# ziatdinovmax/pyroVED

Measured on AMD Instinct MI355X. Metric: images/sec (SVI step), higher is better.
Workload: dtype bf16; 1 GPU; C2 iVAE 28x28 invariances=['r','t'] latent_dim=2 bernoulli, batch 256 per GPU (global 256), bf16 MFMA operands for the hidden-layer contractions (fp32 accumulate; fp32 elsewhere); the guide (fc encoder, sample, split) runs in the decoder launch's prologue in fp32, SVI step = ELBO+grads+Adam; parallelism=dp1

## Files before the change

### pyroved_amd/csrc/pv_elementwise.hip

```cpp
#include "pv_common.h"
#include "pv_kernels.h"
#include "pv_wgrad_small.h"
#include "pv_side.h"
#include "pv_sdec_fused.h"

#define LOG_SQRT_2PI 0.91893853320467274178f
#define BERN_EPS 1.1920928955078125e-07f

__device__ __forceinline__ float block_sum_256(float v, float* sm ) {
  v = pv_wave_sum(v);
  pv_lds_barrier();
  if ((threadIdx.x & 63) == 0) sm[threadIdx.x >> 6] = v;
  pv_lds_barrier();
  return (sm[0] + sm[1]) + (sm[2] + sm[3]);
}

__global__ __launch_bounds__(256) void pv_head_fwd_kernel(PvHead h) {
  __shared__ float sm[4];
  const int total = h.B * h.z_dim;
  float lp = 0.0f, lq = 0.0f;
  for (int e = threadIdx.x; e < total; e += 256) {
    const int b = e / h.z_dim, i = e % h.z_dim;
    const int ldh = h.ldh > 0 ? h.ldh : 2 * h.z_dim;
    const float mu = h.head[(int64_t)b * ldh + i];
// ... 994 lines not shown
}

int pv_latent_bwd_reduce(const PvLatentBwd& p, const float* part, int grid, float* G, const PvFusedOffsets& o, int cd,
                         hipStream_t s, int fmt) {
  if (p.H > 512 || p.lat_in > 64 + (p.K > 0 ? p.K : 0) || p.hb.z_dim > 256 || p.K > 128) return PV_EINVAL;
  PV_LAUNCH_FORK(pv_latent_bwd_reduce_kernel, dim3(pv_fused_reduce_blocks(fmt) + p.hb.B), dim3(256), 0, s, p, part, grid, G, o, cd, fmt);
  PV_LAUNCH_CHECK();
  return 0;
}

__global__ __launch_bounds__(256) void pv_rec_wgrad_kernel(const float* __restrict__ part, int G_, float* __restrict__ Gr, PvFusedOffsets o,
                                                           int cd, int fmt, PvWgradSmall w, PvRecAdam ra, int rwx) {
  __shared__ f32x4 smr[4][64];
  __shared__ float wpart[WG_WAVES][16][17];
  __shared__ float wrpart[WG_WAVES][16];
  const int nred = pv_fused_reduce_blocks(fmt), id = (int)blockIdx.x;
  if (id < nred) { if (!(rwx & 1)) pv_sdec_fused_reduce_block(part, G_, Gr, o, cd, 0, id, smr, fmt, (rwx & 4) ? PvRecAdam{} : ra); return; }
  if (rwx & 2) return;
  pv_wgrad_small_block(w, id - nred, (int)gridDim.x - nred, wpart, wrpart);
}

int pv_rec_wgrad(const float* part, int grid, float* G, const PvFusedOffsets& o, int cd, int fmt, const PvGemm* gs, int n,
                 const PvAdamFuse* adam, const PvFinishArgs* fin, hipStream_t s, unsigned* tick) {
  PvWgradSmall w;
  int guests = 0;
  const int tiles = pv_wgrad_small_fill(w, gs, n, adam, fin, &guests);
  if (tiles < 0) return tiles;
  const int fin_blocks = (fin && fin->scalars) ? 1 : 0;
  if (tick && !fin_blocks) return PV_EINVAL;
  w.tick = tick;
  PvRecAdam ra{};
// ... 114 lines not shown
```

### pyroved_amd/csrc/pv_plan.hip

```cpp
#include "pv_common.h"
#include <algorithm>
#include <stdlib.h>
#include "pv_kernels.h"
#include "pv_sdec_fused.h"
#include "pv_linear.h"
#include "pv_convstack.h"
#include "pv_side.h"
#include "pv_conv.h"

namespace {

struct Carver {
  char* base;
  int64_t off;
  float* take(int64_t nfloats) {
    float* p = base ? (float*)(base + off) : nullptr;
    off += pv_align_up(nfloats * (int64_t)sizeof(float), 256);
    return p;
  }
};

}

int64_t gemm_ws_need(int64_t M, int64_t N, int64_t K) {
// ... 805 lines not shown
  hb.head = L.enc_ext ? p->ext_head : L.head; hb.dhead = L.enc_ext ? p->ext_dhead : L.dhead;
  hb.scale_direct = L.enc_ext ? 1 : 0;
  hb.B = (int)B; hb.z_dim = (int)z; hb.coord_dim = p->coord_dim;
  hb.has_r = p->has_r; hb.has_t = p->has_t; hb.has_s = p->has_s;
  hb.tp0 = p->t_prior[0]; hb.tp1 = p->t_prior[1]; hb.sc_prior = p->sc_prior; hb.beta = p->beta;
  hb.ldh = L.enc_ext ? 0 : (int)plan_head_w(p); hb.kl_mode = p->kl_mode;
  lb.K = (int)K; lb.alpha = L.alpha; lb.beta_disc = p->beta_disc;
  hb.w = p->row_w; lb.row_ll = p->row_elbo ? L.row_ll : nullptr; lb.dzc_out = p->dy ? L.dzc : nullptr;
  static const int chain_env = pv_exp_int("PV_CHAIN", 1) ? 1 : 0;
  const bool chain = chain_env && L.enc_compact && !L.enc_ext && 2 * z + K <= 256;
  if (chain) {
    lb.enc_n = p->n_enc; lb.enc_params = p->params; lb.enc_head = p->head;
    for (int i = 0; i < p->n_enc; ++i) { lb.enc_l[i] = p->enc[i]; lb.enc_act[i] = L.eact[i]; lb.enc_dp[i] = L.edp[i]; }
  }
  static const int ab_tail = pv_exp_int("PV_FOLD_CHAIN", 1);
  const int rec_fmt = p->fused >= 2 ? pv_sdec_fused_bf16_record_fmt(p->fused == 2, R / FD_UNIT, p->dec_kernel) : PV_REC_ROWMAJOR;
  const PvGemm wz = wgrad_problem(L.dhz, H, zin, ldz, G + p->fc_latent.w_off, G + p->fc_coord.b_off, S, lat_in, H);
  PvGemm tail_probs[4];
  int tail_np = -1;
  if (ab_tail && want_grads && chain && f.part_rs && f.dhz_out && f.dzc_out && K == 0 && H == FD_H && !p->row_w &&
      p->kl_mode == PV_KL_SAMPLED &&
      !p->row_elbo && !p->dy && p->head.out_dim <= 16 && p->n_enc == 2 && p->enc[0].out_dim == FD_H && p->enc[1].in_dim == FD_H &&
      p->enc[1].out_dim == FD_H && p->head.in_dim == FD_H) {
    tail_np = compact_wgrad_problems(p, L, &wz, 1, tail_probs);
    if (tail_np > 0 && adam) {
      auto lsz = [](const pv_layer& l) { return (int64_t)l.in_dim * l.out_dim + (l.b_off >= 0 ? l.out_dim : 0); };
      int64_t want = lsz(p->head) + lsz(p->fc_coord) + lsz(p->fc_latent) + lsz(p->out);
      for (int i = 0; i < p->n_enc; ++i) want += lsz(p->enc[i]);
      for (int i = 0; i < p->n_dec; ++i) want += lsz(p->dec[i]);
      int64_t cov = 2 * (int64_t)H * H + (int64_t)H * (3 + p->coord_dim) + 1;
      for (int i = 0; i < tail_np; ++i) cov += (int64_t)tail_probs[i].M * tail_probs[i].N + (tail_probs[i].rowsumA ? tail_probs[i].M : 0);
// ... 465 lines not shown
```

### pyroved_amd/csrc/pv_sdec_fused.h

```cpp
#pragma once
#include "pv_common.h"

#define FD_H 128
#define FD_UNIT 16
#define FD_WAVES 8
#define FD_REC (2 * FD_H * FD_H + 14 * FD_H)
#define PV_RS_W 8
#define FB_WIMG_BYTES (4 * FD_H * FD_H * 2 + 256)

struct PvFused {
  const float* x;
  const float* grid;
  const float* tp;
  const float* hz;
  float hz_scale;
  const float *Wc, *bc;
  const float *W1, *b1;
  const float *W2, *b2;
  const float *wo, *bo;
  float* llrow;
  float* loc;
  float* rowtp;
  float* part_hz;
  float* part_rs;
// ... 70 lines not shown
int pv_sdec_fused_w8x3_launch(const PvFused& f, int grid, bool grads, hipStream_t s, int waves);
int64_t pv_sdec_fused_w8x3_park_bytes(int grid);
int pv_sdec_fused_w8h_launch(const PvFused& f, int grid, bool ds, hipStream_t s);
int64_t pv_sdec_fused_bf16_park_bytes(bool x3, int64_t units, int grid, int sel);
int pv_sdec_fused_bf16_waves(bool x3, int64_t units, int sel);
int pv_sdec_fused_bf16_record_fmt(bool x3, int64_t units, int sel);
bool pv_sdec_fused_sel_valid(int fused, int sel);
struct PvFusedOffsets { int64_t W1, b1, W2, b2, Wc, wo, bo; };
int pv_sdec_fused_reduce(const float* part, int grid, float* G, const PvFusedOffsets& o, int cd, int dwo_slots,
                         hipStream_t s);

#define PV_FUSED_REDUCE_BLOCKS (((2 * FD_H * FD_H + 5 * FD_H + 1 + 3) / 4 + 63) / 64)
#define PV_REC_ROWMAJOR 0
#define PV_REC_LANE_F32 1
#define PV_REC_LANE_BF16 2
#define PV_FUSED_REDUCE_VEC_BLOCKS (((5 * FD_H + 1 + 3) / 4 + 63) / 64)
#define PV_FUSED_REDUCE_MAT_BLOCKS_F32 ((2 * FD_H * FD_H / 4) / 64)
#define PV_FUSED_REDUCE_MAT_BLOCKS_BF16 ((2 * (FD_H / 2) * FD_H / 4) / 64)
__host__ __device__ inline int pv_fused_reduce_mat_blocks(int fmt) {
  return fmt == PV_REC_LANE_BF16 ? PV_FUSED_REDUCE_MAT_BLOCKS_BF16 : PV_FUSED_REDUCE_MAT_BLOCKS_F32;
}
__host__ __device__ inline int pv_fused_reduce_blocks(int fmt) {
  return fmt == PV_REC_ROWMAJOR ? PV_FUSED_REDUCE_BLOCKS : pv_fused_reduce_mat_blocks(fmt) + PV_FUSED_REDUCE_VEC_BLOCKS;
}
#ifndef PV_RED_UNROLL
#define PV_RED_UNROLL 8
#endif
struct PvRecAdam { PvAdamFuse a; int on; };
__device__ __forceinline__ void pv_rec_out(float* __restrict__ Gr, int idx, float v, const PvRecAdam& ad) {
  if (ad.on) pv_adam_update(ad.a.p, ad.a.g, ad.a.m, ad.a.v, (Gr - ad.a.g) + idx, v, ad.a.b1, ad.a.b2, ad.a.eps, ad.a.step_size, ad.a.bc2_sqrt);
  else Gr[idx] = v;
}
template <int FMT>
__device__ __forceinline__ void pv_sdec_fused_reduce_block_lane(const float* __restrict__ part, int G_, float* __restrict__ Gr,
                                                                const PvFusedOffsets& o, int block, f32x4 (*sm)[64],
                                                                const PvRecAdam& ad = PvRecAdam{}) {
  const int c = threadIdx.x & 63, sl = threadIdx.x >> 6;
  const int per = (G_ + 3) / 4;
  const int w0 = sl * per, w1 = min(G_, w0 + per);
  const float* pbase = part + 4 * (block * 64 + c);
  f32x4 a = {0.0f, 0.0f, 0.0f, 0.0f}, b = {0.0f, 0.0f, 0.0f, 0.0f};
  if (FMT == PV_REC_LANE_BF16) {
    typedef unsigned int u32x4_ __attribute__((ext_vector_type(4)));
#pragma unroll PV_RED_UNROLL
    for (int w = w0; w < w1; ++w) {
      const u32x4_ v = *reinterpret_cast<const u32x4_*>(pbase + (int64_t)w * FD_REC);
      a[0] += __uint_as_float(v[0] << 16); a[1] += __uint_as_float(v[0] & 0xffff0000u);
      a[2] += __uint_as_float(v[1] << 16); a[3] += __uint_as_float(v[1] & 0xffff0000u);
      b[0] += __uint_as_float(v[2] << 16); b[1] += __uint_as_float(v[2] & 0xffff0000u);
      b[2] += __uint_as_float(v[3] << 16); b[3] += __uint_as_float(v[3] & 0xffff0000u);
    }
  } else {
#pragma unroll PV_RED_UNROLL
    for (int w = w0; w < w1; ++w) a += *reinterpret_cast<const f32x4*>(pbase + (int64_t)w * FD_REC);
  }
  sm[sl][c] = a;
  __syncthreads();
  const f32x4 ta = (sm[0][c] + sm[1][c]) + (sm[2][c] + sm[3][c]);
  f32x4 tb = b;
  if (FMT == PV_REC_LANE_BF16) {
    __syncthreads();
    sm[sl][c] = b;
    __syncthreads();
    tb = (sm[0][c] + sm[1][c]) + (sm[2][c] + sm[3][c]);
  }
  if (sl != 0) return;
  const int r = c & 15, q = c >> 4;
  if (FMT == PV_REC_LANE_BF16) {
    const int oo = block & 3, s_ = (block >> 2) & 1, wave = block >> 3, jp = wave >> 1, kh = wave & 1;
    const int row0 = 32 * jp + 16 * (s_ ^ kh) + 4 * q, col = 64 * kh + 16 * oo + r;
#pragma unroll
    for (int i = 0; i < 4; ++i) {
      pv_rec_out(Gr, o.W1 + (row0 + i) * FD_H + col, ta[i], ad);
      pv_rec_out(Gr, o.W2 + (row0 + i) * FD_H + col, tb[i], ad);
    }
  } else {
    const int kb = block & 7, s_ = (block >> 3) & 1, wave = (block >> 4) & 3, m = block >> 6;
    const int row0 = 16 * (2 * wave + s_) + 4 * q, col = 16 * kb + r;
    const int dst = m == 0 ? o.W1 : o.W2;
#pragma unroll
    for (int i = 0; i < 4; ++i) pv_rec_out(Gr, dst + (row0 + i) * FD_H + col, ta[i], ad);
  }
}
__device__ __forceinline__ void pv_sdec_fused_reduce_block(const float* __restrict__ part, int G_,
                                                           float* __restrict__ Gr, const PvFusedOffsets& o, int cd,
                                                           int dwo_slots, int block, f32x4 (*sm)[64], int fmt = PV_REC_ROWMAJOR,
                                                           const PvRecAdam& ad = PvRecAdam{}) {
  const int HH = FD_H * FD_H;
  const int total = 2 * HH + 5 * FD_H + 1;
  const int c = threadIdx.x & 63, sl = threadIdx.x >> 6;
  if (fmt != PV_REC_ROWMAJOR && block < pv_fused_reduce_mat_blocks(fmt)) {
    if (fmt == PV_REC_LANE_BF16) pv_sdec_fused_reduce_block_lane<PV_REC_LANE_BF16>(part, G_, Gr, o, block, sm, ad);
    else pv_sdec_fused_reduce_block_lane<PV_REC_LANE_F32>(part, G_, Gr, o, block, sm, ad);
    return;
  }
  const int e = fmt != PV_REC_ROWMAJOR ? 2 * HH + ((block - pv_fused_reduce_mat_blocks(fmt)) * 64 + c) * 4 : (block * 64 + c) * 4;
  const int per = (G_ + 3) / 4;
  const int w0 = sl * per, w1 = min(G_, w0 + per);
  f32x4 v = {0.0f, 0.0f, 0.0f, 0.0f};
  if (e < total) {
    const bool slots = dwo_slots && e >= 2 * HH + 4 * FD_H && e < 2 * HH + 5 * FD_H;
    if (slots) {
      for (int w = w0; w < w1; ++w) {
        const float* p8 = part + (int64_t)w * FD_REC + 2 * HH + 6 * FD_H + (e - (2 * HH + 4 * FD_H));
        f32x4 a = {0.0f, 0.0f, 0.0f, 0.0f};
        for (int k = 0; k < FD_WAVES; ++k) a += *reinterpret_cast<const f32x4*>(p8 + k * FD_H);
        v += a;
// ... 31 lines not shown
```

### pyroved_amd/csrc/pv_sdec_fused_w8.hip

```cpp
#include "pv_sdec_fused.h"
#include "pv_fb_layout.h"
#include "pv_kernels.h"
#include <stdlib.h>

typedef short short4_ __attribute__((ext_vector_type(4)));
typedef short short8_ __attribute__((ext_vector_type(8)));
typedef __attribute__((address_space(3))) short4_ lds_short4;

#define W8_WAVES 8
#define W8_ROWS (W8_WAVES * FD_UNIT)
#define W8_THREADS (64 * W8_WAVES)
#define LDS2 144
#define W8_ARR (W8_ROWS * LDS2)
#define W8_ARR_BYTES (2 * W8_ARR)
#define WO_W1 0
#define WO_W2 IMG_BYTES
#define WO_SA (2 * IMG_BYTES)
#define WO_SB (WO_SA + W8_ARR_BYTES)
#define WO_VEC (WO_SB + W8_ARR_BYTES)
#define WO_ATAB (WO_VEC + 3 * FD_H * 4)
#define WO_TTAB (WO_ATAB + 8 * 64 * 8)
#define WO_INFO (WO_TTAB + 4 * 64 * 16)
#define WO_RED (WO_INFO + 3 * W8_ROWS * 4)
#define WO_CHZ (WO_RED + 256)
// ... 349 lines not shown
  return h;
}
__device__ __forceinline__ f32x4 w8_mul_dtanh4(const f32x4& d, const bf16x4& hb) {
  const f32x4 t = w8_f32_of(hb);
  return d * (t * t - 1.0f);
}

#define WF_H1 WO_SA
#define WF_H2 (WF_H1 + 512)
#define WF_HD (WF_H2 + 512)
#define WF_P (WF_HD + 512)
#define WF_P_WAVE (64 * 17 * 4)
static_assert(WF_P + W8_WAVES * WF_P_WAVE <= WO_VEC, "guide scratch fits in the staging arrays");
#include "pv_gemv16.h"

#define W8_COOP_SPINS 4096
__device__ unsigned w8_coop_late_total;
extern "C" int pv_debug_coop_late_count(unsigned* out) {
  return (int)hipMemcpyFromSymbol(out, HIP_SYMBOL(w8_coop_late_total), sizeof(unsigned));
}
template <bool GRADS, int LIK, int FOLDK>
__global__ __launch_bounds__(W8_THREADS) void pv_sdec_w8_kernel(PvFused f, PvEncFold e) {
  constexpr bool FOLD = FOLDK != 0, CHAIN = FOLDK >= 2, COOP = FOLDK == 3;
  extern __shared__ __attribute__((aligned(16))) char smb[];
  const int tid = threadIdx.x, lane0 = tid & 63, lane = lane0, r = lane & 15, q = lane >> 4;
  const int wave = __builtin_amdgcn_readfirstlane(tid >> 6);
  const int g = blockIdx.x, G = gridDim.x;
  const unsigned lds0 = __builtin_amdgcn_readfirstlane((unsigned)(size_t)smb);
  const __bf16* W1h = reinterpret_cast<const __bf16*>(smb + WO_W1);
  const __bf16* W2h = reinterpret_cast<const __bf16*>(smb + WO_W2);
// ... 359 lines not shown
  const int xun = (int)f.x_units;
  struct Pos { int unit, b, loc, xu; };
  auto pos_of = [&](int unit_) {
    Pos p_;
    p_.unit = unit_; p_.b = unit_ / upb; p_.loc = unit_ - p_.b * upb; p_.xu = xun > 0 ? unit_ % xun : unit_;
    return p_;
  };
  auto advance = [&](Pos& p_, int by) {
    p_.unit += by; p_.loc += by; p_.xu += by;
    while (p_.loc >= upb) { p_.loc -= upb; ++p_.b; }
    if (xun > 0) { while (p_.xu >= xun) p_.xu -= xun; }
  };
  const bool has_tail = W8_TAIL && ((u_hi - u_lo) & (W8_WAVES - 1)) == 1;
  const int u_end = has_tail ? u_hi - 1 : u_hi;
  const Pos pos_lo = pos_of(has_tail ? u_end : u_lo);
  Pos pos_cur = pos_of(u_lo + wave < u_end ? u_lo + wave : (has_tail ? u_end : u_lo));
  Pos pos_nx = pos_cur;
  float sw_next = 1.0f;
  auto x_of = [&](const Pos& p_) -> float {
    if (f.sw) sw_next = f.sw[p_.b];
    return f.x[(int64_t)p_.xu * FD_UNIT + r];
  };
  float xv_next = x_of(pos_cur);
  float* chz = reinterpret_cast<float*>(smb + WO_CHZ) + wave * FD_H;
  float* ctp = reinterpret_cast<float*>(smb + WO_CTP) + wave * 64;
  float* cgr = reinterpret_cast<float*>(smb + WO_CGR) + wave * 64;
  auto fetch_unit_inputs = [&](const Pos& p_) {
    const int n0 = p_.loc * FD_UNIT;
    w8_glds4(f.hz + (int64_t)p_.b * FD_H + lane, lds0 + WO_CHZ + wave * (FD_H * 4));
    w8_glds4(f.hz + (int64_t)p_.b * FD_H + 64 + lane, lds0 + WO_CHZ + wave * (FD_H * 4) + 256);
    w8_glds4(f.tp + (int64_t)p_.b * 8 + (lane & 7), lds0 + WO_CTP + wave * 256);
    w8_glds4(f.grid + (int64_t)n0 * f.cd + (lane & (16 * f.cd - 1)), lds0 + WO_CGR + wave * 256);
  };
  fetch_unit_inputs(pos_cur);
  const W8Addr wad = w8_addr(r, q);
  int tile_no = -1;
  for (int ut = u_lo; ut < u_end; ut += W8_WAVES) {
    ++tile_no;
    (void)tile_no;
    asm volatile("; W8_TILE_BEGIN");
    W8_STAMP(0);
    const int nact = (u_end - ut) < W8_WAVES ? (u_end - ut) : W8_WAVES;
    if (ut + W8_WAVES + wave < u_end) advance(pos_nx, W8_WAVES);
    else pos_nx = pos_lo;
    int opq = 0;
    asm volatile("" : "+v"(opq));
    const int lane = lane0 | opq, r = lane & 15, q = lane >> 4;
    const float* wos = vec;
    const float* b1s = vec + FD_H;
    const float* b2s = vec + 2 * FD_H;
// ... 128 lines not shown
      w8_colsum_mfma(sA, pA, bw, accS, wave, r, q);
#pragma unroll
      for (int jb = 0; jb < 8; ++jb) tC[jb] = tC[jb] * dlda;
      w8_cvt8(tC, pA);
    }
    asm volatile("; W8_P4_dwo_done");
    W8_STAMP(4);
    w8_stage_store(sA, pA, 16 * wave + r, q);
    w8_stage_store(sB, h1b, 16 * wave + r, q);
    __syncthreads();
    asm volatile("; W8_P5_bar1");
    W8_STAMP(5);
    w8_wgrad_consume(sA, sB, accW2, accB2, wave, r, q, ksteps);
    asm volatile("; W8_P6_cons2");
    W8_STAMP(6);
    bf16x4 p0[8];
    {
      w8_layer_dgrad(W2h, pA, tC, wad);
      w8_mul_dtanh(tC, h1b);
      w8_cvt8(tC, pA);
      asm volatile("; W8_P7_dgrad2");
    W8_STAMP(7);
      w8_layer_dgrad(W1h, pA, tC, wad);
      w8_mul_dtanh(tC, h0b);
      w8_cvt8(tC, p0);
    }
    asm volatile("; W8_P8_dgrad1");
    W8_STAMP(8);
    __syncthreads();
    W8_STAMP(9);
// ... 34 lines not shown
    w8_stage_store(sA, pA, 16 * wave + r, q);
    w8_stage_store(sB, h0b, 16 * wave + r, q);
    __syncthreads();
    asm volatile("; W8_P10_bar3");
    W8_STAMP(10);
    w8_wgrad_consume(sA, sB, accW1, accB1, wave, r, q, ksteps);
    asm volatile("; W8_P11_cons1");
    W8_STAMP(11);
    __syncthreads();
    asm volatile("; W8_P13_bar4");
    W8_STAMP(13);
    W8_STAMP(14);
    asm volatile("; W8_TILE_END");
  }

  if (has_tail) {
    asm volatile("; W8_TAIL_BEGIN");
    const int lane = lane0, r = lane & 15, q = lane >> 4;
    const float* wos = vec;
    const float* b1s = vec + FD_H;
    const float* b2s = vec + 2 * FD_H;
    const int unit = u_end, bu = pos_cur.b;
    const int64_t row = (int64_t)unit * FD_UNIT + r;
    float x0, x1, u0c, u1c, sc;
    w8_wait_vm0();
    {
      const float* t = ctp;
      const float* gr = cgr;
      if (f.cd == 2) {
        const float gx = gr[2 * r], gy = gr[2 * r + 1];
        u0c = gx * t[0] - gy * t[1];
        u1c = gx * t[1] + gy * t[0];
        sc = t[2];
        x0 = u0c * sc + t[3];
        x1 = u1c * sc + t[4];
      } else {
        u0c = gr[r]; u1c = 0.0f; sc = 1.0f;
        x0 = u0c + t[3]; x1 = 0.0f;
      }
    }
    const float xv = xv_next, swv = sw_next;
    float* inf_x0 = info + 16 * wave;
    float* inf_x1 = info + W8_ROWS + 16 * wave;
    float* inf_dl = info + 2 * W8_ROWS + 16 * wave;
    bf16x4 h0b[8], h1b[8], own0, own1;
    {
      bf16x4 bx = w8_zero4();
      {
        const float v = q == 0 ? x0 : x1;
        __bf16 vh, vl;
        fb_split(v, vh, vl);
        const __bf16 one = (__bf16)1.0f;
        if (q < 2) { bx[0] = vh; bx[1] = vl; bx[2] = vh; }
        else if (q == 2) { bx[0] = one; bx[1] = one; }
      }
      f32x4 t0 = *reinterpret_cast<const f32x4*>(chz + 16 * wave + 4 * q);
      if (f.hz_scale == 0.0f) t0 = t0 * W8_C;
      const bf16x4 aop = (reinterpret_cast<const bf16x4*>(smb + WO_ATAB) + lane)[64 * wave];
      if (GRADS && q == 0) { inf_x0[r] = x0; inf_x1[r] = x1; }
      t0 = w8_mfma16(aop, bx, t0);
      own0 = w8_cvt4(w8_tanh4(t0));
      w8_xchg_put(smb, 0, own0, wave, lane);
    }
    __syncthreads();
    w8_xchg_get(smb, 0, h0b, lane);
    own1 = w8_cvt4(w8_tanh4(w8_tail_fwd(W1h, b1s, h0b, wad, wave, q)));
    w8_xchg_put(smb, 1, own1, wave, lane);
    __syncthreads();
    w8_xchg_get(smb, 1, h1b, lane);
    f32x4 gq;
    float dlda = 0.0f;
    {
      const f32x4 t2 = w8_tanh4(w8_tail_fwd(W2h, b2s, h1b, wad, wave, q));
      const f32x4 wv = *reinterpret_cast<const f32x4*>(wos + 16 * wave + 4 * q);
      const f32x4 pw = t2 * wv;
      const float part = w8_sum_q((pw[0] + pw[1]) + (pw[2] + pw[3]));
      if (GRADS) {
        w8_xchg_put(smb, 2, w8_cvt4(t2), wave, lane);
        gq = wv - wv * (t2 * t2);
      }
      float* tlog = reinterpret_cast<float*>(smb + WO_TLOG);
      if (q == 0) tlog[16 * wave + r] = part;
      __syncthreads();
      float a = bo;
      {
        float sacc = 0.0f;
#pragma unroll
        for (int w = 0; w < W8_WAVES; ++w) sacc += tlog[16 * w + r];
        a += sacc;
      }
      float ll, locv;
      if (LIK == PV_LIK_BERNOULLI) {
        const float pr = w8_rcp(1.0f + w8_exp(-a));
        const float pc = fminf(fmaxf(pr, BERN_EPS), 1.0f - BERN_EPS);
        const float lpc = w8_log(pc), l1pc = w8_log(1.0f - pc);
        const float lg = lpc - l1pc;
        ll = -(fmaxf(lg, 0.0f) - lg * xv - fmaxf(lpc, l1pc));
        const float mask = (pr >= BERN_EPS && pr <= 1.0f - BERN_EPS) ? 1.0f : 0.0f;
        dlda = (pc - xv) * mask;
        locv = pr;
      } else if (LIK == PV_LIK_CBERNOULLI) {
        pv_cbern(a, xv, ll, dlda, locv);
      } else {
        const float pr = f.sigmoid_out ? w8_rcp(1.0f + w8_exp(-a)) : a;
        const float d = xv - pr;
        ll = -(d * d) / (2.0f * f.sig * f.sig) - w8_log(f.sig) - LOG_SQRT_2PI;
        dlda = -d / (f.sig * f.sig) * (f.sigmoid_out ? pr * (1.0f - pr) : 1.0f);
        locv = pr;
      }
      dlda *= swv;
      if (q == 0) {
        if (wave == 0) {
          if (a_llrow) a_llrow[row] = ll;
          if (a_loc) a_loc[row] = locv;
          if (GRADS) dbo += dlda;
        }
        if (GRADS) inf_dl[r] = dlda;
      }
    }
    if (GRADS) {
      bf16x4 pA[8];
      w8_xchg_put(smb, 3, w8_cvt4(gq * dlda), wave, lane);
      __syncthreads();
      w8_xchg_get(smb, 3, pA, lane);
      if (wave == 0) {
        w8_stage_store(sA, pA, r, q);
        w8_stage_store(sB, h1b, r, q);
      } else if (wave == 1) {
        bf16x4 z8[8];
#pragma unroll
        for (int jb = 0; jb < 8; ++jb) z8[jb] = w8_zero4();
        w8_stage_store(sA, z8, 16 + r, q);
        w8_stage_store(sB, h1b, 16 + r, q);
      } else if (wave == 3) {
        bf16x4 h2b[8];
        w8_xchg_get(smb, 2, h2b, lane);
        w8_wait_lgkm0();
        const f32x4 d4 = *reinterpret_cast<const f32x4*>(inf_dl + 4 * q);
        bf16x4 bw = w8_zero4();
#pragma unroll
        for (int i = 0; i < 4; ++i) {
          __bf16 hi, lo;
          fb_split(d4[i], hi, lo);
          bw[i] = r == 3 ? hi : (r == 4 ? lo : (__bf16)0.0f);
        }
        w8_colsum_mfma(sA, h2b, bw, accS, wave, r, q);
      }
      const f32x4 d1 = w8_mul_dtanh4(w8_tail_dgrad(W2h, pA, wad, wave, r), own1);
      w8_xchg_put(smb, 4, w8_cvt4(d1), wave, lane);
      __syncthreads();
      w8_xchg_get(smb, 4, pA, lane);
      w8_wgrad_consume(sA, sB, accW2, accB2, wave, r, q, 1);
      const f32x4 d0 = w8_mul_dtanh4(w8_tail_dgrad(W1h, pA, wad, wave, r), own0);
      w8_xchg_put(smb, 5, w8_cvt4(d0), wave, lane);
      __syncthreads();
      if (wave == 0) {
        w8_stage_store(sA, pA, r, q);
        w8_stage_store(sB, h0b, r, q);
      } else if (wave == 1) {
        bf16x4 z8[8];
#pragma unroll
        for (int jb = 0; jb < 8; ++jb) z8[jb] = w8_zero4();
        w8_stage_store(sA, z8, 16 + r, q);
        w8_stage_store(sB, h0b, 16 + r, q);
      } else if (wave == 2) {
        bf16x4 p0[8];
        w8_xchg_get(smb, 5, p0, lane);
        f32x4 dd = {0.0f, 0.0f, 0.0f, 0.0f};
        const bf16x8* ttab = reinterpret_cast<const bf16x8*>(smb + WO_TTAB) + lane;
#pragma unroll
        for (int mm = 0; mm < 4; ++mm) dd = MFMA32(ttab[64 * mm], w8_cat(p0[2 * mm], p0[2 * mm + 1]), dd);
        if (q == 0) {
          const float d0_ = (dd[0] + dd[1]) * W8_RC2, d1_ = (dd[2] + dd[3]) * W8_RC2;
          a_rowtp[row] = sc * (d1_ * u0c - d0_ * u1c);
          a_rowtp[a_M + row] = d0_ * u0c + d1_ * u1c;
          a_rowtp[2 * a_M + row] = d0_;
          a_rowtp[3 * a_M + row] = d1_;
        }
      } else if (wave == 3) {
        bf16x4 p0[8];
        w8_xchg_get(smb, 5, p0, lane);
        if (bu != cur_b) {
          if (cur_b >= 0) flush_hz(cur_b);
          cur_b = bu;
        }
        const f32x4 a0 = *reinterpret_cast<const f32x4*>(inf_x0 + 4 * q);
        const f32x4 a1 = *reinterpret_cast<const f32x4*>(inf_x1 + 4 * q);
        bf16x4 bc_ = w8_zero4();
        const bool use1 = r == 2 || r == 6, lo_col = r >= 5;
#pragma unroll
        for (int i = 0; i < 4; ++i) {
          __bf16 hi, lo;
          fb_split(use1 ? a1[i] : a0[i], hi, lo);
          __bf16 v = lo_col ? lo : hi;
          if (r == 0) v = (__bf16)1.0f;
          if (r == 3 || r == 4 || r > 6) v = (__bf16)0.0f;
          bc_[i] = v;
        }
        w8_colsum_mfma(sA, p0, bc_, accS, wave, r, q);
      }
      __syncthreads();
      w8_wgrad_consume(sA, sB, accW1, accB1, wave, r, q, 1);
    }
    asm volatile("; W8_TAIL_END");
  }
  if (!GRADS) return;
  W8_STAMP_K(2);

  const PvEncFoldArg ep_ = pv_kernarg_fold();
  const bool own_dhz = FOLD && f.dhz_out != nullptr;
  if (cur_b >= 0 && !own_dhz) flush_hz(cur_b);
  W8_STAMP_E(0);
  __syncthreads();
  W8_STAMP_E(1);
  float rsv[2][5] = {{0.0f, 0.0f, 0.0f, 0.0f, 0.0f}, {0.0f, 0.0f, 0.0f, 0.0f, 0.0f}};
  const bool fold_rs = FOLD && f.part_rs && f.N <= 2 * W8_THREADS && f.N % 2 == 0;
  if (fold_rs) {
    const int64_t r0 = (int64_t)g * f.N;
    if (2 * tid < f.N) {
// ... 31 lines not shown
    if (lane < ep_->z_dim && wave < 2) {
      ch_z = ldc(ep_->z + (int64_t)g * ep_->z_dim + lane);
      ch_sig = ldc(ep_->z_scale + (int64_t)g * ep_->z_dim + lane);
      ch_ep = ep_->eps[(int64_t)g * ep_->z_dim + lane];
      ch_sp = ldc(ep_->head_out + (int64_t)g * ep_->ldh + ep_->z_dim + lane);
    }
  }
  W8_STAMP_E(11);
  {
    const int jp = wave >> 1, kh = wave & 1;
    auto pack2 = [](float a, float b) {
      typedef __bf16 bf2_ __attribute__((ext_vector_type(2)));
      bf2_ h; h[0] = (__bf16)a; h[1] = (__bf16)b;
      return __builtin_bit_cast(unsigned, h);
    };
    if (f.ablate & 1024) {
#pragma unroll
      for (int s_ = 0; s_ < 2; ++s_)
#pragma unroll
        for (int o = 0; o < 4; ++o)
#pragma unroll
          for (int i = 0; i < 4; ++i) {
            const int e = (32 * jp + 16 * (s_ ^ kh) + 4 * q + i) * FD_H + 64 * kh + 16 * o + r;
            rec[e] = accW1[s_][o][i] * -W8_RC;
            rec[FD_H * FD_H + e] = accW2[s_][o][i];
          }
    } else {
      typedef unsigned int u32x4_ __attribute__((ext_vector_type(4)));
      u32x4_* rec4 = reinterpret_cast<u32x4_*>(rec);
#pragma unroll
      for (int s_ = 0; s_ < 2; ++s_)
#pragma unroll
        for (int o = 0; o < 4; ++o) {
          u32x4_ v;
          v[0] = pack2(accW1[s_][o][0] * -W8_RC, accW1[s_][o][1] * -W8_RC);
          v[1] = pack2(accW1[s_][o][2] * -W8_RC, accW1[s_][o][3] * -W8_RC);
          v[2] = pack2(accW2[s_][o][0], accW2[s_][o][1]);
          v[3] = pack2(accW2[s_][o][2], accW2[s_][o][3]);
          rec4[((wave * 2 + s_) * 4 + o) * 64 + lane] = v;
        }
    }
    if (r == 0) {
      const int j0 = 32 * jp + 16 * kh;
#pragma unroll
      for (int i = 0; i < 4; ++i) {
        rec[2 * FD_H * FD_H + j0 + 4 * q + i] = accB1[i] * -W8_RC;
        rec[2 * FD_H * FD_H + FD_H + j0 + 4 * q + i] = accB2[i];
      }
    }
  }
  W8_STAMP_E(12);
  {
    float* scr = reinterpret_cast<float*>(smb + WO_SA);
#pragma unroll
    for (int jb = 0; jb < 8; ++jb)
      *reinterpret_cast<f32x4*>(scr + ((wave * 16 + r) * FD_H) + 16 * jb + 4 * q) = accS[jb];
  }
// ... 177 lines not shown
```

Before: 2.686 million images/s.

## Run fused decoder tail unit first and split W2 record store early

In the folded w8 decoder, the leftover tail unit now runs before the main tile loop instead of after it. The W2 gradient partials are then written to the per-block record as soon as the last tile's W2 accumulation finishes, rather than at the epilogue. A new split record format (separate W1/W2 halves) and a permuted block ordering in the reduce/wgrad kernel let the W2 reductions get scheduled ahead of the W1 ones. The aim is to shorten the epilogue critical path and overlap record stores with remaining compute, at the cost of a more complex record layout and extra barriers.

```diff
diff --git a/pyroved_amd/csrc/pv_elementwise.hip b/pyroved_amd/csrc/pv_elementwise.hip
--- a/pyroved_amd/csrc/pv_elementwise.hip
+++ b/pyroved_amd/csrc/pv_elementwise.hip
@@ -1032,7 +1032,9 @@
   __shared__ f32x4 smr[4][64];
   __shared__ float wpart[WG_WAVES][16][17];
   __shared__ float wrpart[WG_WAVES][16];
-  const int nred = pv_fused_reduce_blocks(fmt), id = (int)blockIdx.x;
+  const int nred = pv_fused_reduce_blocks(fmt);
+  const int id = fmt == PV_REC_LANE_BF16_SPLIT ? pv_rec_wgrad_order((int)blockIdx.x, (int)gridDim.x, nred, w.fin_scalars ? 1 : 0)
+                                               : (int)blockIdx.x;
   if (id < nred) { if (!(rwx & 1)) pv_sdec_fused_reduce_block(part, G_, Gr, o, cd, 0, id, smr, fmt, (rwx & 4) ? PvRecAdam{} : ra); return; }
   if (rwx & 2) return;
   pv_wgrad_small_block(w, id - nred, (int)gridDim.x - nred, wpart, wrpart);
diff --git a/pyroved_amd/csrc/pv_plan.hip b/pyroved_amd/csrc/pv_plan.hip
--- a/pyroved_amd/csrc/pv_plan.hip
+++ b/pyroved_amd/csrc/pv_plan.hip
@@ -843,7 +843,8 @@
     for (int i = 0; i < p->n_enc; ++i) { lb.enc_l[i] = p->enc[i]; lb.enc_act[i] = L.eact[i]; lb.enc_dp[i] = L.edp[i]; }
   }
   static const int ab_tail = pv_exp_int("PV_FOLD_CHAIN", 1);
-  const int rec_fmt = p->fused >= 2 ? pv_sdec_fused_bf16_record_fmt(p->fused == 2, R / FD_UNIT, p->dec_kernel) : PV_REC_ROWMAJOR;
+  int rec_fmt = p->fused >= 2 ? pv_sdec_fused_bf16_record_fmt(p->fused == 2, R / FD_UNIT, p->dec_kernel) : PV_REC_ROWMAJOR;
+  if (fold && rec_fmt == PV_REC_LANE_BF16) rec_fmt = PV_REC_LANE_BF16_SPLIT;
   const PvGemm wz = wgrad_problem(L.dhz, H, zin, ldz, G + p->fc_latent.w_off, G + p->fc_coord.b_off, S, lat_in, H);
   PvGemm tail_probs[4];
   int tail_np = -1;
diff --git a/pyroved_amd/csrc/pv_sdec_fused.h b/pyroved_amd/csrc/pv_sdec_fused.h
--- a/pyroved_amd/csrc/pv_sdec_fused.h
+++ b/pyroved_amd/csrc/pv_sdec_fused.h
@@ -108,14 +108,27 @@
 #define PV_REC_ROWMAJOR 0
 #define PV_REC_LANE_F32 1
 #define PV_REC_LANE_BF16 2
+#define PV_REC_LANE_BF16_SPLIT 3
 #define PV_FUSED_REDUCE_VEC_BLOCKS (((5 * FD_H + 1 + 3) / 4 + 63) / 64)
 #define PV_FUSED_REDUCE_MAT_BLOCKS_F32 ((2 * FD_H * FD_H / 4) / 64)
 #define PV_FUSED_REDUCE_MAT_BLOCKS_BF16 ((2 * (FD_H / 2) * FD_H / 4) / 64)
 __host__ __device__ inline int pv_fused_reduce_mat_blocks(int fmt) {
-  return fmt == PV_REC_LANE_BF16 ? PV_FUSED_REDUCE_MAT_BLOCKS_BF16 : PV_FUSED_REDUCE_MAT_BLOCKS_F32;
+  return (fmt == PV_REC_LANE_BF16 || fmt == PV_REC_LANE_BF16_SPLIT) ? PV_FUSED_REDUCE_MAT_BLOCKS_BF16 : PV_FUSED_REDUCE_MAT_BLOCKS_F32;
 }
 __host__ __device__ inline int pv_fused_reduce_blocks(int fmt) {
   return fmt == PV_REC_ROWMAJOR ? PV_FUSED_REDUCE_BLOCKS : pv_fused_reduce_mat_blocks(fmt) + PV_FUSED_REDUCE_VEC_BLOCKS;
+}
+__host__ __device__ inline int pv_rec_wgrad_order(int p, int total, int nred, int nfin) {
+  const int half = PV_FUSED_REDUCE_MAT_BLOCKS_BF16 / 2, ntile = total - nred - nfin;
+  if (p < nfin) return total - 1;
+  p -= nfin;
+  if (p < half) return half + p;
+  if (p == half) return nred - 1;
+  p -= half + 1;
+  if (p < ntile) return nred + p;
+  p -= ntile;
+  if (p < half) return p;
+  return 2 * half + (p - half);
 }
 #ifndef PV_RED_UNROLL
 #define PV_RED_UNROLL 8
@@ -134,7 +147,8 @@
   const int w0 = sl * per, w1 = min(G_, w0 + per);
   const float* pbase = part + 4 * (block * 64 + c);
   f32x4 a = {0.0f, 0.0f, 0.0f, 0.0f}, b = {0.0f, 0.0f, 0.0f, 0.0f};
-  if (FMT == PV_REC_LANE_BF16) {
+  constexpr bool PACKED = FMT == PV_REC_LANE_BF16 || FMT == PV_REC_LANE_BF16_SPLIT;
+  if (PACKED) {
     typedef unsigned int u32x4_ __attribute__((ext_vector_type(4)));
 #pragma unroll PV_RED_UNROLL
     for (int w = w0; w < w1; ++w) {
@@ -152,7 +166,7 @@
   __syncthreads();
   const f32x4 ta = (sm[0][c] + sm[1][c]) + (sm[2][c] + sm[3][c]);
   f32x4 tb = b;
-  if (FMT == PV_REC_LANE_BF16) {
+  if (PACKED) {
     __syncthreads();
     sm[sl][c] = b;
     __syncthreads();
@@ -160,7 +174,16 @@
   }
   if (sl != 0) return;
   const int r = c & 15, q = c >> 4;
-  if (FMT == PV_REC_LANE_BF16) {
+  if (FMT == PV_REC_LANE_BF16_SPLIT) {
+    const int oo = 2 * (block & 1) + (c >> 5), s_ = (block >> 1) & 1, wave = (block >> 2) & 7, m = block >> 5, jp = wave >> 1, kh = wave & 1;
+    const int ln = 2 * (c & 31), row0 = 32 * jp + 16 * (s_ ^ kh) + 4 * (ln >> 4), col = 64 * kh + 16 * oo + (ln & 15);
+    const int dst = m == 0 ? o.W1 : o.W2;
+#pragma unroll
+    for (int i = 0; i < 4; ++i) {
+      pv_rec_out(Gr, dst + (row0 + i) * FD_H + col, ta[i], ad);
+      pv_rec_out(Gr, dst + (row0 + i) * FD_H + col + 1, tb[i], ad);
+    }
+  } else if (FMT == PV_REC_LANE_BF16) {
     const int oo = block & 3, s_ = (block >> 2) & 1, wave = block >> 3, jp = wave >> 1, kh = wave & 1;
     const int row0 = 32 * jp + 16 * (s_ ^ kh) + 4 * q, col = 64 * kh + 16 * oo + r;
 #pragma unroll
@@ -185,6 +208,7 @@
   const int c = threadIdx.x & 63, sl = threadIdx.x >> 6;
   if (fmt != PV_REC_ROWMAJOR && block < pv_fused_reduce_mat_blocks(fmt)) {
     if (fmt == PV_REC_LANE_BF16) pv_sdec_fused_reduce_block_lane<PV_REC_LANE_BF16>(part, G_, Gr, o, block, sm, ad);
+    else if (fmt == PV_REC_LANE_BF16_SPLIT) pv_sdec_fused_reduce_block_lane<PV_REC_LANE_BF16_SPLIT>(part, G_, Gr, o, block, sm, ad);
     else pv_sdec_fused_reduce_block_lane<PV_REC_LANE_F32>(part, G_, Gr, o, block, sm, ad);
     return;
   }
diff --git a/pyroved_amd/csrc/pv_sdec_fused_w8.hip b/pyroved_amd/csrc/pv_sdec_fused_w8.hip
--- a/pyroved_amd/csrc/pv_sdec_fused_w8.hip
+++ b/pyroved_amd/csrc/pv_sdec_fused_w8.hip
@@ -387,6 +387,43 @@
 static_assert(WF_P + W8_WAVES * WF_P_WAVE <= WO_VEC, "guide scratch fits in the staging arrays");
 #include "pv_gemv16.h"
 
+#if defined(__HIP_DEVICE_COMPILE__)
+typedef const __attribute__((address_space(4))) PvFused* PvFusedArg;
+__device__ __forceinline__ PvFusedArg w8_kernarg_fused() {
+  PvFusedArg p = (PvFusedArg)__builtin_amdgcn_kernarg_segment_ptr();
+  asm volatile("" : "+s"(p));
+  return p;
+}
+#else
+typedef const PvFused* PvFusedArg;
+__device__ inline PvFusedArg w8_kernarg_fused() { return nullptr; }
+#endif
+__device__ __forceinline__ unsigned w8_pack2(float a, float b) {
+  typedef __bf16 bf2_ __attribute__((ext_vector_type(2)));
+  bf2_ h; h[0] = (__bf16)a; h[1] = (__bf16)b;
+  return __builtin_bit_cast(unsigned, h);
+}
+__device__ __forceinline__ void w8_store_rec_half(float* rec, int m, const f32x4 (&acc)[2][4], float mul, int wave, int lane) {
+  typedef unsigned int u32x2_ __attribute__((ext_vector_type(2)));
+  u32x2_* rec2 = reinterpret_cast<u32x2_*>(rec) + ((m * W8_WAVES + wave) * 8) * 64 + lane;
+#pragma unroll
+  for (int s_ = 0; s_ < 2; ++s_)
+#pragma unroll
+    for (int o = 0; o < 4; ++o) {
+      u32x2_ v;
+      v[0] = w8_pack2(acc[s_][o][0] * mul, acc[s_][o][1] * mul);
+      v[1] = w8_pack2(acc[s_][o][2] * mul, acc[s_][o][3] * mul);
+      rec2[(s_ * 4 + o) * 64] = v;
+    }
+}
+__device__ __forceinline__ void w8_store_rec_bias(float* rec, int seg, const f32x4& acc, float mul, int wave, int r, int q) {
+  if (r == 0) {
+    const int j0 = 32 * (wave >> 1) + 16 * (wave & 1);
+#pragma unroll
+    for (int i = 0; i < 4; ++i) rec[2 * FD_H * FD_H + seg * FD_H + j0 + 4 * q + i] = acc[i] * mul;
+  }
+}
+
 #define W8_COOP_SPINS 4096
 __device__ unsigned w8_coop_late_total;
 extern "C" int pv_debug_coop_late_count(unsigned* out) {
@@ -776,7 +813,9 @@
   const bool has_tail = W8_TAIL && ((u_hi - u_lo) & (W8_WAVES - 1)) == 1;
   const int u_end = has_tail ? u_hi - 1 : u_hi;
   const Pos pos_lo = pos_of(has_tail ? u_end : u_lo);
-  Pos pos_cur = pos_of(u_lo + wave < u_end ? u_lo + wave : (has_tail ? u_end : u_lo));
+  const bool tail_first = FOLD && has_tail;
+  const Pos pos_t0 = pos_of(u_lo + wave < u_end ? u_lo + wave : (has_tail ? u_end : u_lo));
+  Pos pos_cur = tail_first ? pos_lo : pos_t0;
   Pos pos_nx = pos_cur;
   float sw_next = 1.0f;
   auto x_of = [&](const Pos& p_) -> float {
@@ -796,6 +835,10 @@
   };
   fetch_unit_inputs(pos_cur);
   const W8Addr wad = w8_addr(r, q);
+  if constexpr (FOLD) {
+    if (has_tail)
+#include "pv_sdec_w8_tail.inc"
+  }
   int tile_no = -1;
   for (int ut = u_lo; ut < u_end; ut += W8_WAVES) {
     ++tile_no;
@@ -954,6 +997,16 @@
     w8_wgrad_consume(sA, sB, accW2, accB2, wave, r, q, ksteps);
     asm volatile("; W8_P6_cons2");
     W8_STAMP(6);
+    if constexpr (FOLD) {
+      if (ut + W8_WAVES >= u_end) {
+        const PvFusedArg fk = w8_kernarg_fused();
+        if (!(fk->ablate & 1024)) {
+          float* rec_ = fk->part + (int64_t)g * FD_REC;
+          w8_store_rec_half(rec_, 1, accW2, 1.0f, wave, lane);
+          w8_store_rec_bias(rec_, 1, accB2, 1.0f, wave, r, q);
+        }
+      }
+    }
     bf16x4 p0[8];
     {
       w8_layer_dgrad(W2h, pA, tC, wad);
@@ -1018,195 +1071,9 @@
     asm volatile("; W8_TILE_END");
   }
 
-  if (has_tail) {
-    asm volatile("; W8_TAIL_BEGIN");
-    const int lane = lane0, r = lane & 15, q = lane >> 4;
-    const float* wos = vec;
-    const float* b1s = vec + FD_H;
-    const float* b2s = vec + 2 * FD_H;
-    const int unit = u_end, bu = pos_cur.b;
-    const int64_t row = (int64_t)unit * FD_UNIT + r;
-    float x0, x1, u0c, u1c, sc;
-    w8_wait_vm0();
-    {
-      const float* t = ctp;
-      const float* gr = cgr;
-      if (f.cd == 2) {
-        const float gx = gr[2 * r], gy = gr[2 * r + 1];
-        u0c = gx * t[0] - gy * t[1];
-        u1c = gx * t[1] + gy * t[0];
-        sc = t[2];
-        x0 = u0c * sc + t[3];
-        x1 = u1c * sc + t[4];
-      } else {
-        u0c = gr[r]; u1c = 0.0f; sc = 1.0f;
-        x0 = u0c + t[3]; x1 = 0.0f;
-      }
-    }
-    const float xv = xv_next, swv = sw_next;
-    float* inf_x0 = info + 16 * wave;
-    float* inf_x1 = info + W8_ROWS + 16 * wave;
-    float* inf_dl = info + 2 * W8_ROWS + 16 * wave;
-    bf16x4 h0b[8], h1b[8], own0, own1;
-    {
-      bf16x4 bx = w8_zero4();
-      {
-        const float v = q == 0 ? x0 : x1;
-        __bf16 vh, vl;
-        fb_split(v, vh, vl);
-        const __bf16 one = (__bf16)1.0f;
-        if (q < 2) { bx[0] = vh; bx[1] = vl; bx[2] = vh; }
-        else if (q == 2) { bx[0] = one; bx[1] = one; }
-      }
-      f32x4 t0 = *reinterpret_cast<const f32x4*>(chz + 16 * wave + 4 * q);
-      if (f.hz_scale == 0.0f) t0 = t0 * W8_C;
-      const bf16x4 aop = (reinterpret_cast<const bf16x4*>(smb + WO_ATAB) + lane)[64 * wave];
-      if (GRADS && q == 0) { inf_x0[r] = x0; inf_x1[r] = x1; }
-      t0 = w8_mfma16(aop, bx, t0);
-      own0 = w8_cvt4(w8_tanh4(t0));
-      w8_xchg_put(smb, 0, own0, wave, lane);
-    }
-    __syncthreads();
-    w8_xchg_get(smb, 0, h0b, lane);
-    own1 = w8_cvt4(w8_tanh4(w8_tail_fwd(W1h, b1s, h0b, wad, wave, q)));
-    w8_xchg_put(smb, 1, own1, wave, lane);
-    __syncthreads();
-    w8_xchg_get(smb, 1, h1b, lane);
-    f32x4 gq;
-    float dlda = 0.0f;
-    {
-      const f32x4 t2 = w8_tanh4(w8_tail_fwd(W2h, b2s, h1b, wad, wave, q));
-      const f32x4 wv = *reinterpret_cast<const f32x4*>(wos + 16 * wave + 4 * q);
-      const f32x4 pw = t2 * wv;
-      const float part = w8_sum_q((pw[0] + pw[1]) + (pw[2] + pw[3]));
-      if (GRADS) {
-        w8_xchg_put(smb, 2, w8_cvt4(t2), wave, lane);
-        gq = wv - wv * (t2 * t2);
-      }
-      float* tlog = reinterpret_cast<float*>(smb + WO_TLOG);
-      if (q == 0) tlog[16 * wave + r] = part;
-      __syncthreads();
-      float a = bo;
-      {
-        float sacc = 0.0f;
-#pragma unroll
-        for (int w = 0; w < W8_WAVES; ++w) sacc += tlog[16 * w + r];
-        a += sacc;
-      }
-      float ll, locv;
-      if (LIK == PV_LIK_BERNOULLI) {
-        const float pr = w8_rcp(1.0f + w8_exp(-a));
-        const float pc = fminf(fmaxf(pr, BERN_EPS), 1.0f - BERN_EPS);
-        const float lpc = w8_log(pc), l1pc = w8_log(1.0f - pc);
-        const float lg = lpc - l1pc;
-        ll = -(fmaxf(lg, 0.0f) - lg * xv - fmaxf(lpc, l1pc));
-        const float mask = (pr >= BERN_EPS && pr <= 1.0f - BERN_EPS) ? 1.0f : 0.0f;
-        dlda = (pc - xv) * mask;
-        locv = pr;
-      } else if (LIK == PV_LIK_CBERNOULLI) {
-        pv_cbern(a, xv, ll, dlda, locv);
-      } else {
-        const float pr = f.sigmoid_out ? w8_rcp(1.0f + w8_exp(-a)) : a;
-        const float d = xv - pr;
-        ll = -(d * d) / (2.0f * f.sig * f.sig) - w8_log(f.sig) - LOG_SQRT_2PI;
-        dlda = -d / (f.sig * f.sig) * (f.sigmoid_out ? pr * (1.0f - pr) : 1.0f);
-        locv = pr;
-      }
-      dlda *= swv;
-      if (q == 0) {
-        if (wave == 0) {
-          if (a_llrow) a_llrow[row] = ll;
-          if (a_loc) a_loc[row] = locv;
-          if (GRADS) dbo += dlda;
-        }
-        if (GRADS) inf_dl[r] = dlda;
-      }
-    }
-    if (GRADS) {
-      bf16x4 pA[8];
-      w8_xchg_put(smb, 3, w8_cvt4(gq * dlda), wave, lane);
-      __syncthreads();
-      w8_xchg_get(smb, 3, pA, lane);
-      if (wave == 0) {
-        w8_stage_store(sA, pA, r, q);
-        w8_stage_store(sB, h1b, r, q);
-      } else if (wave == 1) {
-        bf16x4 z8[8];
-#pragma unroll
-        for (int jb = 0; jb < 8; ++jb) z8[jb] = w8_zero4();
-        w8_stage_store(sA, z8, 16 + r, q);
-        w8_stage_store(sB, h1b, 16 + r, q);
-      } else if (wave == 3) {
-        bf16x4 h2b[8];
-        w8_xchg_get(smb, 2, h2b, lane);
-        w8_wait_lgkm0();
-        const f32x4 d4 = *reinterpret_cast<const f32x4*>(inf_dl + 4 * q);
-        bf16x4 bw = w8_zero4();
-#pragma unroll
-        for (int i = 0; i < 4; ++i) {
-          __bf16 hi, lo;
-          fb_split(d4[i], hi, lo);
-          bw[i] = r == 3 ? hi : (r == 4 ? lo : (__bf16)0.0f);
-        }
-        w8_colsum_mfma(sA, h2b, bw, accS, wave, r, q);
-      }
-      const f32x4 d1 = w8_mul_dtanh4(w8_tail_dgrad(W2h, pA, wad, wave, r), own1);
-      w8_xchg_put(smb, 4, w8_cvt4(d1), wave, lane);
-      __syncthreads();
-      w8_xchg_get(smb, 4, pA, lane);
-      w8_wgrad_consume(sA, sB, accW2, accB2, wave, r, q, 1);
-      const f32x4 d0 = w8_mul_dtanh4(w8_tail_dgrad(W1h, pA, wad, wave, r), own0);
-      w8_xchg_put(smb, 5, w8_cvt4(d0), wave, lane);
-      __syncthreads();
-      if (wave == 0) {
-        w8_stage_store(sA, pA, r, q);
-        w8_stage_store(sB, h0b, r, q);
-      } else if (wave == 1) {
-        bf16x4 z8[8];
-#pragma unroll
-        for (int jb = 0; jb < 8; ++jb) z8[jb] = w8_zero4();
-        w8_stage_store(sA, z8, 16 + r, q);
-        w8_stage_store(sB, h0b, 16 + r, q);
-      } else if (wave == 2) {
-        bf16x4 p0[8];
-        w8_xchg_get(smb, 5, p0, lane);
-        f32x4 dd = {0.0f, 0.0f, 0.0f, 0.0f};
-        const bf16x8* ttab = reinterpret_cast<const bf16x8*>(smb + WO_TTAB) + lane;
-#pragma unroll
-        for (int mm = 0; mm < 4; ++mm) dd = MFMA32(ttab[64 * mm], w8_cat(p0[2 * mm], p0[2 * mm + 1]), dd);
-        if (q == 0) {
-          const float d0_ = (dd[0] + dd[1]) * W8_RC2, d1_ = (dd[2] + dd[3]) * W8_RC2;
-          a_rowtp[row] = sc * (d1_ * u0c - d0_ * u1c);
-          a_rowtp[a_M + row] = d0_ * u0c + d1_ * u1c;
-          a_rowtp[2 * a_M + row] = d0_;
-          a_rowtp[3 * a_M + row] = d1_;
-        }
-      } else if (wave == 3) {
-        bf16x4 p0[8];
-        w8_xchg_get(smb, 5, p0, lane);
-        if (bu != cur_b) {
-          if (cur_b >= 0) flush_hz(cur_b);
-          cur_b = bu;
-        }
-        const f32x4 a0 = *reinterpret_cast<const f32x4*>(inf_x0 + 4 * q);
-        const f32x4 a1 = *reinterpret_cast<const f32x4*>(inf_x1 + 4 * q);
-        bf16x4 bc_ = w8_zero4();
-        const bool use1 = r == 2 || r == 6, lo_col = r >= 5;
-#pragma unroll
-        for (int i = 0; i < 4; ++i) {
-          __bf16 hi, lo;
-          fb_split(use1 ? a1[i] : a0[i], hi, lo);
-          __bf16 v = lo_col ? lo : hi;
-          if (r == 0) v = (__bf16)1.0f;
-          if (r == 3 || r == 4 || r > 6) v = (__bf16)0.0f;
-          bc_[i] = v;
-        }
-        w8_colsum_mfma(sA, p0, bc_, accS, wave, r, q);
-      }
-      __syncthreads();
-      w8_wgrad_consume(sA, sB, accW1, accB1, wave, r, q, 1);
-    }
-    asm volatile("; W8_TAIL_END");
+  if constexpr (!FOLD) {
+    if (has_tail)
+#include "pv_sdec_w8_tail.inc"
   }
   if (!GRADS) return;
   W8_STAMP_K(2);
@@ -1268,7 +1135,15 @@
       bf2_ h; h[0] = (__bf16)a; h[1] = (__bf16)b;
       return __builtin_bit_cast(unsigned, h);
     };
-    if (f.ablate & 1024) {
+    const bool split = FOLD && !(f.ablate & 1024);
+    if (split) {
+      w8_store_rec_half(rec, 0, accW1, -W8_RC, wave, lane);
+      w8_store_rec_bias(rec, 0, accB1, -W8_RC, wave, r, q);
+      if (u_end <= u_lo) {
+        w8_store_rec_half(rec, 1, accW2, 1.0f, wave, lane);
+        w8_store_rec_bias(rec, 1, accB2, 1.0f, wave, r, q);
+      }
+    } else if (f.ablate & 1024) {
 #pragma unroll
       for (int s_ = 0; s_ < 2; ++s_)
 #pragma unroll
@@ -1294,7 +1169,7 @@
           rec4[((wave * 2 + s_) * 4 + o) * 64 + lane] = v;
         }
     }
-    if (r == 0) {
+    if (!split && r == 0) {
       const int j0 = 32 * jp + 16 * kh;
 #pragma unroll
       for (int i = 0; i < 4; ++i) {
diff --git a/pyroved_amd/csrc/pv_sdec_w8_tail.inc b/pyroved_amd/csrc/pv_sdec_w8_tail.inc
--- /dev/null
+++ b/pyroved_amd/csrc/pv_sdec_w8_tail.inc
@@ -0,0 +1,197 @@
+  {
+    asm volatile("; W8_TAIL_BEGIN");
+    const int lane = lane0, r = lane & 15, q = lane >> 4;
+    const float* wos = vec;
+    const float* b1s = vec + FD_H;
+    const float* b2s = vec + 2 * FD_H;
+    const int unit = u_end, bu = pos_cur.b;
+    const int64_t row = (int64_t)unit * FD_UNIT + r;
+    float x0, x1, u0c, u1c, sc;
+    w8_wait_vm0();
+    {
+      const float* t = ctp;
+      const float* gr = cgr;
+      if (f.cd == 2) {
+        const float gx = gr[2 * r], gy = gr[2 * r + 1];
+        u0c = gx * t[0] - gy * t[1];
+        u1c = gx * t[1] + gy * t[0];
+        sc = t[2];
+        x0 = u0c * sc + t[3];
+        x1 = u1c * sc + t[4];
+      } else {
+        u0c = gr[r]; u1c = 0.0f; sc = 1.0f;
+        x0 = u0c + t[3]; x1 = 0.0f;
+      }
+    }
+    const float xv = xv_next, swv = sw_next;
+    float* inf_x0 = info + 16 * wave;
+    float* inf_x1 = info + W8_ROWS + 16 * wave;
+    float* inf_dl = info + 2 * W8_ROWS + 16 * wave;
+    bf16x4 h0b[8], h1b[8], own0, own1;
+    {
+      bf16x4 bx = w8_zero4();
+      {
+        const float v = q == 0 ? x0 : x1;
+        __bf16 vh, vl;
+        fb_split(v, vh, vl);
+        const __bf16 one = (__bf16)1.0f;
+        if (q < 2) { bx[0] = vh; bx[1] = vl; bx[2] = vh; }
+        else if (q == 2) { bx[0] = one; bx[1] = one; }
+      }
+      f32x4 t0 = *reinterpret_cast<const f32x4*>(chz + 16 * wave + 4 * q);
+      if (f.hz_scale == 0.0f) t0 = t0 * W8_C;
+      const bf16x4 aop = (reinterpret_cast<const bf16x4*>(smb + WO_ATAB) + lane)[64 * wave];
+      if (GRADS && q == 0) { inf_x0[r] = x0; inf_x1[r] = x1; }
+      t0 = w8_mfma16(aop, bx, t0);
+      own0 = w8_cvt4(w8_tanh4(t0));
+      w8_xchg_put(smb, 0, own0, wave, lane);
+    }
+    if constexpr (FOLD) {
+      fetch_unit_inputs(pos_t0);
+      xv_next = x_of(pos_t0);
+      pos_cur = pos_t0;
+      pos_nx = pos_t0;
+    }
+    __syncthreads();
+    w8_xchg_get(smb, 0, h0b, lane);
+    own1 = w8_cvt4(w8_tanh4(w8_tail_fwd(W1h, b1s, h0b, wad, wave, q)));
+    w8_xchg_put(smb, 1, own1, wave, lane);
+    __syncthreads();
+    w8_xchg_get(smb, 1, h1b, lane);
+    f32x4 gq;
+    float dlda = 0.0f;
+    {
+      const f32x4 t2 = w8_tanh4(w8_tail_fwd(W2h, b2s, h1b, wad, wave, q));
+      const f32x4 wv = *reinterpret_cast<const f32x4*>(wos + 16 * wave + 4 * q);
+      const f32x4 pw = t2 * wv;
+      const float part = w8_sum_q((pw[0] + pw[1]) + (pw[2] + pw[3]));
+      if (GRADS) {
+        w8_xchg_put(smb, 2, w8_cvt4(t2), wave, lane);
+        gq = wv - wv * (t2 * t2);
+      }
+      float* tlog = reinterpret_cast<float*>(smb + WO_TLOG);
+      if (q == 0) tlog[16 * wave + r] = part;
+      __syncthreads();
+      float a = bo;
+      {
+        float sacc = 0.0f;
+#pragma unroll
+        for (int w = 0; w < W8_WAVES; ++w) sacc += tlog[16 * w + r];
+        a += sacc;
+      }
+      float ll, locv;
+      if (LIK == PV_LIK_BERNOULLI) {
+        const float pr = w8_rcp(1.0f + w8_exp(-a));
+        const float pc = fminf(fmaxf(pr, BERN_EPS), 1.0f - BERN_EPS);
+        const float lpc = w8_log(pc), l1pc = w8_log(1.0f - pc);
+        const float lg = lpc - l1pc;
+        ll = -(fmaxf(lg, 0.0f) - lg * xv - fmaxf(lpc, l1pc));
+        const float mask = (pr >= BERN_EPS && pr <= 1.0f - BERN_EPS) ? 1.0f : 0.0f;
+        dlda = (pc - xv) * mask;
+        locv = pr;
+      } else if (LIK == PV_LIK_CBERNOULLI) {
+        pv_cbern(a, xv, ll, dlda, locv);
+      } else {
+        const float pr = f.sigmoid_out ? w8_rcp(1.0f + w8_exp(-a)) : a;
+        const float d = xv - pr;
+        ll = -(d * d) / (2.0f * f.sig * f.sig) - w8_log(f.sig) - LOG_SQRT_2PI;
+        dlda = -d / (f.sig * f.sig) * (f.sigmoid_out ? pr * (1.0f - pr) : 1.0f);
+        locv = pr;
+      }
+      dlda *= swv;
+      if (q == 0) {
+        if (wave == 0) {
+          if (a_llrow) a_llrow[row] = ll;
+          if (a_loc) a_loc[row] = locv;
+          if (GRADS) dbo += dlda;
+        }
+        if (GRADS) inf_dl[r] = dlda;
+      }
+    }
+    if (GRADS) {
+      bf16x4 pA[8];
+      w8_xchg_put(smb, 3, w8_cvt4(gq * dlda), wave, lane);
+      __syncthreads();
+      w8_xchg_get(smb, 3, pA, lane);
+      if (wave == 0) {
+        w8_stage_store(sA, pA, r, q);
+        w8_stage_store(sB, h1b, r, q);
+      } else if (wave == 1) {
+        bf16x4 z8[8];
+#pragma unroll
+        for (int jb = 0; jb < 8; ++jb) z8[jb] = w8_zero4();
+        w8_stage_store(sA, z8, 16 + r, q);
+        w8_stage_store(sB, h1b, 16 + r, q);
+      } else if (wave == 3) {
+        bf16x4 h2b[8];
+        w8_xchg_get(smb, 2, h2b, lane);
+        w8_wait_lgkm0();
+        const f32x4 d4 = *reinterpret_cast<const f32x4*>(inf_dl + 4 * q);
+        bf16x4 bw = w8_zero4();
+#pragma unroll
+        for (int i = 0; i < 4; ++i) {
+          __bf16 hi, lo;
+          fb_split(d4[i], hi, lo);
+          bw[i] = r == 3 ? hi : (r == 4 ? lo : (__bf16)0.0f);
+        }
+        w8_colsum_mfma(sA, h2b, bw, accS, wave, r, q);
+      }
+      const f32x4 d1 = w8_mul_dtanh4(w8_tail_dgrad(W2h, pA, wad, wave, r), own1);
+      w8_xchg_put(smb, 4, w8_cvt4(d1), wave, lane);
+      __syncthreads();
+      w8_xchg_get(smb, 4, pA, lane);
+      w8_wgrad_consume(sA, sB, accW2, accB2, wave, r, q, 1);
+      const f32x4 d0 = w8_mul_dtanh4(w8_tail_dgrad(W1h, pA, wad, wave, r), own0);
+      w8_xchg_put(smb, 5, w8_cvt4(d0), wave, lane);
+      __syncthreads();
+      if (wave == 0) {
+        w8_stage_store(sA, pA, r, q);
+        w8_stage_store(sB, h0b, r, q);
+      } else if (wave == 1) {
+        bf16x4 z8[8];
+#pragma unroll
+        for (int jb = 0; jb < 8; ++jb) z8[jb] = w8_zero4();
+        w8_stage_store(sA, z8, 16 + r, q);
+        w8_stage_store(sB, h0b, 16 + r, q);
+      } else if (wave == 2) {
+        bf16x4 p0[8];
+        w8_xchg_get(smb, 5, p0, lane);
+        f32x4 dd = {0.0f, 0.0f, 0.0f, 0.0f};
+        const bf16x8* ttab = reinterpret_cast<const bf16x8*>(smb + WO_TTAB) + lane;
+#pragma unroll
+        for (int mm = 0; mm < 4; ++mm) dd = MFMA32(ttab[64 * mm], w8_cat(p0[2 * mm], p0[2 * mm + 1]), dd);
+        if (q == 0) {
+          const float d0_ = (dd[0] + dd[1]) * W8_RC2, d1_ = (dd[2] + dd[3]) * W8_RC2;
+          a_rowtp[row] = sc * (d1_ * u0c - d0_ * u1c);
+          a_rowtp[a_M + row] = d0_ * u0c + d1_ * u1c;
+          a_rowtp[2 * a_M + row] = d0_;
+          a_rowtp[3 * a_M + row] = d1_;
+        }
+      } else if (wave == 3) {
+        bf16x4 p0[8];
+        w8_xchg_get(smb, 5, p0, lane);
+        if (bu != cur_b) {
+          if (cur_b >= 0) flush_hz(cur_b);
+          cur_b = bu;
+        }
+        const f32x4 a0 = *reinterpret_cast<const f32x4*>(inf_x0 + 4 * q);
+        const f32x4 a1 = *reinterpret_cast<const f32x4*>(inf_x1 + 4 * q);
+        bf16x4 bc_ = w8_zero4();
+        const bool use1 = r == 2 || r == 6, lo_col = r >= 5;
+#pragma unroll
+        for (int i = 0; i < 4; ++i) {
+          __bf16 hi, lo;
+          fb_split(use1 ? a1[i] : a0[i], hi, lo);
+          __bf16 v = lo_col ? lo : hi;
+          if (r == 0) v = (__bf16)1.0f;
+          if (r == 3 || r == 4 || r > 6) v = (__bf16)0.0f;
+          bc_[i] = v;
+        }
+        w8_colsum_mfma(sA, p0, bc_, accS, wave, r, q);
+      }
+      __syncthreads();
+      w8_wgrad_consume(sA, sB, accW1, accB1, wave, r, q, 1);
+      if constexpr (FOLD) __syncthreads();
+    }
+    asm volatile("; W8_TAIL_END");
+  }
```

Measured after the change: 2.653 million images/s. -1.2%, worse.
